# Medical-Image-Analysis-Laboratory/fetal_t2mapping

Measured on AMD Instinct MI355X. Metric: Mvoxel/s T2 fit, 256³×8TE 3-param LM, 1/2/4/8 GPU; % HBM roofline, higher is better.
Workload: dtype f64

## Files before the change

fetal_t2mapping_amd/csrc/t2fit_kernels.hip:

```cpp
#include <hip/hip_runtime.h>

#include <algorithm>
#include <atomic>
#include <cstdlib>
#include <string>

#include "t2fit_config.h"
#include "t2fit_diag.h"
#include "t2fit_dispatch.h"
#include "t2fit_error.h"
#include "t2fit_launch.h"
#include "t2fit_support.h"

using namespace t2fit;

namespace {

constexpr int kLdsStride = kBlock + 1;
#ifndef T2_SAMPLE_LOAD
#define T2_SAMPLE_LOAD(p) (*(p))
#endif
#ifndef T2_WAVE_HINT
#define T2_WAVE_HINT 2
#endif
// ... 209 lines not shown
        finite = finite && t2_finite(sv);
      }
    }
    ObjCtx c;
    c.P = &P;
    c.y = EchoView{col, kLoglinTile};
    double lb[3], ub[3];
    const bool feasible = lane_bounds(P, y0[q], lb, ub);
    LaneResult r;
    r.nit = 0; r.nfev = 0; r.fun = NAN;
    if (!feasible) {
      r.x[0] = NAN; r.x[1] = NAN; r.x[2] = 0.0;
      r.status = T2FIT_ST_INFEASIBLE;
    } else if (!finite) {
      r.x[0] = t2_clip(P.x0[0], lb[0], ub[0]); r.x[1] = t2_clip(P.x0[1], lb[1], ub[1]); r.x[2] = 0.0;
      r.status = T2FIT_ST_NONFINITE;
    } else {
      loglin_solve(c, lb, ub, want_fun, r);
    }
    LaneOutputs o;
    lane_epilogue(c, r, o, kExtras && m.r2 != nullptr, kExtras && m.se != nullptr);
    o_t2[q] = o.t2; o_k[q] = o.k; o_res[q] = o.res;
    if constexpr (kExtras) {
      if (m.r2) m.r2[v] = o.r2;
      if (m.se) m.se[v] = o.se;
      if (m.fun) m.fun[v] = o.fun;
      if (m.nit) m.nit[v] = o.nit;
      if (m.status) m.status[v] = o.status;
      if (m.xd) { m.xd[3 * v] = r.x[0]; m.xd[3 * v + 1] = r.x[1]; m.xd[3 * v + 2] = r.x[2]; }
      if (m.fund) m.fund[v] = r.fun;
    }
  }
  *reinterpret_cast<float4*>(m.t2 + v0) = make_float4(o_t2[0], o_t2[1], o_t2[2], o_t2[3]);
  *reinterpret_cast<float4*>(m.k + v0) = make_float4(o_k[0], o_k[1], o_k[2], o_k[3]);
  *reinterpret_cast<float4*>(m.sigma + v0) = make_float4(0.0f, 0.0f, 0.0f, 0.0f);
  *reinterpret_cast<float4*>(m.res + v0) = make_float4(o_res[0], o_res[1], o_res[2], o_res[3]);
}

constexpr int kChunkLarge = 256;
constexpr int kChunkSmall = 64;
constexpr int kQueueCap = 64 + kChunkLarge;

template <int MODEL, int NTE = 0, int HOME = PAIRS_LDS> struct LbfgsbLane {
  using Solver = Lbfgsb<MODEL, NTE, HOME>;
  using WaveWg = LbfgsbLane<MODEL, NTE, MODEL == T2FIT_MODEL_GAUSSIAN ? PAIRS_LDS
                                         : MODEL == T2FIT_MODEL_RICIAN ? PAIRS_GLOBAL : PAIRS_REG>;
  static constexpr bool kGlobalPart = Solver::kPairGlobal;
  static constexpr int NP = Solver::N;
  static constexpr int kNte = NTE;
  static constexpr int kHistDoubles = Solver::M * Solver::PAIR_L;
  static constexpr int kWavesPerSimd = 1;
  static constexpr bool kWaveWgOk = true;
#ifndef T2_WAVE_HINT_2PAR
#define T2_WAVE_HINT_2PAR 3
#endif
  static constexpr int kWaveWgHint = MODEL == T2FIT_MODEL_GAUSSIAN ? T2_WAVE_HINT_2PAR : kWaveHint;
  static constexpr int kRefillMin = MODEL == T2FIT_MODEL_RICIAN ? 4 : 8;
  static constexpr bool kSplit = true;
  __device__ static void init(Solver& s, const ObjCtx&, const double* x0, const double* lb, const double* ub,
                              double* hist, int hstride, double* ghist) { s.init(x0, lb, ub, hist, hstride, ghist, 64); }
  __device__ static void result(const Solver& s, const ObjCtx&, LaneResult& r) { s.result(r); }
  template <int J> __device__ static void take_sample(Solver& s, float y) {
    if constexpr (NTE > 0 && J < NTE) s.ys[J] = y;
  }
};
template <typename T, int NPAR, int NTE = 0> struct LmLaneAdaptor {
  using Solver = LmLane<T, NPAR, NTE>;
  using WaveWg = LmLaneAdaptor<T, NPAR, NTE>;
  static constexpr bool kGlobalPart = false;
  static constexpr int NP = NPAR;
  static constexpr int kNte = NTE;
  static constexpr int kHistDoubles = 0;
  static constexpr bool kWaveWgOk = false;
  static constexpr int kWaveWgHint = 1;
  static constexpr int kWavesPerSimd = sizeof(T) == 4 ? 4 : 1;
  static constexpr int kRefillMin = 24;
  static constexpr bool kSplit = false;
  __device__ static void init(Solver& s, const ObjCtx& c, const double* x0, const double* lb, const double* ub,
                              double*, int, double*) { s.init(c, x0, lb, ub); }
  __device__ static void result(const Solver& s, const ObjCtx& c, LaneResult& r) { s.result(c, r); }
  template <int J> __device__ static void take_sample(Solver&, float) {}
};

template <class A, int kChunk, bool kTrace, bool kExtras, int kWg = kBlock, bool kRegs = false>
__device__ __forceinline__ void persistent_fit(const LaneParams& P, const float* __restrict__ echoes, int layout,
                                               const uint8_t* __restrict__ mask, int64_t n_vox, const DevMaps& m,
                                               unsigned long long* next_chunk, int refill_min, int take, double* ghist_all) {
  extern __shared__ float lds[];
  constexpr int NP = A::NP;
  constexpr bool kWaveWg = kRegs;
  static_assert(kRegs ? (kChunk == 64 && A::kNte > 0 && A::kNte <= 8) : kWg == kBlock,
                "workgroup of 256 lanes, or waves taking 64-voxel chunks with the samples in registers");
  constexpr int kStride = kWaveWg ? 64 : kLdsStride;
  const int lane = threadIdx.x & 63, wave = threadIdx.x >> 6;
  float* col = lds + threadIdx.x;
  double* hist = reinterpret_cast<double*>(lds + (kWaveWg ? 0 : ((P.n_te * kStride + 1) & ~1))) + threadIdx.x;
  uint32_t* queue = reinterpret_cast<uint32_t*>(hist - threadIdx.x + A::kHistDoubles * kWg) + wave * kQueueCap;
  double* ghist = nullptr;
  if constexpr (A::kGlobalPart)
    ghist = ghist_all + ((size_t)blockIdx.x * (kWg / 64) + wave) * (A::Solver::M * 64) + lane;
  uint32_t qv = 0;
  const unsigned long long lt_mask = lane == 0 ? 0ull : (~0ull >> (64 - lane));
  const EchoView y{col, kStride};
  int q_head = 0, q_count = 0;
  bool chunks_left = true;
  bool busy = false, done = false;
  int64_t v = 0;
  typename A::Solver s;
  ObjCtx c;
  c.P = &P;
  c.y = y;
  double box_x0[3], box_lb[3], box_ub[3];
#pragma unroll
  for (int j = 0; j < 3; ++j) { box_x0[j] = P.x0[j]; box_lb[j] = P.lb[j]; box_ub[j] = P.ub[j]; }
  T2_STAMPS_BEGIN(queue - wave * kQueueCap + (kBlock / 64) * kQueueCap, wave, lane, c)
  T2_RECORD_PLACEMENT(next_chunk, blockIdx.x * (kWg / 64) + wave, lane)
  bool parked = false;
  int pend = 0;
  const int kTake = take;
  int64_t base_a = 0;
  int sub_a = 0;
  uint32_t idx_b = 0;
  uint8_t mask_a = 0;
  auto load_mask = [&](int64_t base) -> uint8_t {
    const int64_t vv = base + lane;
    return vv < n_vox ? (mask ? mask[vv] : (uint8_t)1) : (uint8_t)0;
  };
  if constexpr (kWaveWg) {
    uint32_t c0 = 0;
    if (lane == 0) c0 = (uint32_t)atomicAdd(next_chunk, 1ull);
    base_a = (int64_t)__shfl(c0, 0, 64) * (64 * kTake);
    mask_a = load_mask(base_a);
    if (lane == 0) idx_b = (uint32_t)atomicAdd(next_chunk, 1ull);
  }
  for (;;) {
    unsigned long long need = __ballot(!busy);
    if (__popcll(need) >= refill_min || need == ~0ull) {
      do {
      T2_BLK_T0(t_rf)
      if (done) {
        LaneResult r;
        A::result(s, c, r);
        store_fit<kExtras>(m, v, r);
        done = false;
      }
      bool fresh = false;
      if constexpr (kWaveWg) {
        unsigned long long want = need;
        for (;;) {
          if (q_count == 0) {
            if (!chunks_left) break;
            const int64_t base = base_a;
            if (base >= n_vox) { chunks_left = false; break; }
            const int64_t vv = base + lane;
            const bool act = mask_a != 0;
            if (++sub_a < kTake) {
              base_a += 64;
              mask_a = load_mask(base_a);
            } else {
              sub_a = 0;
              base_a = (int64_t)__shfl(idx_b, 0, 64) * (64 * kTake);
              mask_a = load_mask(base_a);
              if (lane == 0) idx_b = (uint32_t)atomicAdd(next_chunk, 1ull);
            }
            const unsigned long long b = __ballot(act);
            q_count = __popcll(b);
            q_head = 0;
            const int dst = act ? __popcll(b & lt_mask) : q_count + __popcll(~b & lt_mask);
            qv = (uint32_t)__builtin_amdgcn_ds_permute(dst << 2, (int)(uint32_t)vv);
            if (vv < n_vox && !act) store_masked<kExtras, true>(m, vv);
            if (q_count == 0) continue;
          }
          const int rank = __popcll(want & lt_mask);
          const uint32_t got = (uint32_t)__builtin_amdgcn_ds_bpermute(((q_head + rank) & 63) << 2, (int)qv);
          if (!busy && rank < q_count) {
            v = (int64_t)got;
            busy = true;
            fresh = true;
          }
          const int n_want = __popcll(want);
          const int taken = n_want < q_count ? n_want : q_count;
          q_head += taken;
          q_count -= taken;
          want = __ballot(!busy);
          if (want == 0ull) break;
        }
      } else {
      const int n_need = __popcll(need);
      while (q_count < n_need && chunks_left) {
        unsigned long long cidx = 0;
        if (lane == 0) cidx = atomicAdd(next_chunk, 1ull);
        cidx = __shfl(cidx, 0, 64);
        const int64_t base = (int64_t)cidx * kChunk;
        if (base >= n_vox) { chunks_left = false; break; }
        if (q_head != 0) {
          uint32_t tmp = 0;
          if (lane < q_count) tmp = queue[q_head + lane];
          if (lane < q_count) queue[lane] = tmp;
          q_head = 0;
        }
        bool act[kChunk / 64];
#pragma unroll
        for (int q = 0; q < kChunk / 64; ++q) {
          const int64_t vv = base + q * 64 + lane;
          act[q] = vv < n_vox && (mask == nullptr || mask[vv] != 0);
        }
#pragma unroll
        for (int q = 0; q < kChunk / 64; ++q) {
          const unsigned long long b = __ballot(act[q]);
          if (act[q]) queue[q_count + __popcll(b & lt_mask)] = (uint32_t)(base + q * 64 + lane);
          q_count += __popcll(b);
        }
#pragma unroll
        for (int q = 0; q < kChunk / 64; ++q) {
          const int64_t vv = base + q * 64 + lane;
          if (vv < n_vox && !act[q]) store_masked<kExtras, true>(m, vv);
        }
      }
      if (!busy) {
        const int rank = __popcll(need & lt_mask);
        if (rank < q_count) {
          v = (int64_t)queue[q_head + rank];
          busy = true;
          fresh = true;
        }
      }
      const int taken = n_need < q_count ? n_need : q_count;
      q_head += taken;
      q_count -= taken;
      }
      if (fresh) {
        bool finite = true;
        float ymax = 0.0f, y0 = 0.0f;
        const int n_te = A::kNte > 0 ? A::kNte : P.n_te;
        float first8[8] = {};
        for (int i0 = 0; i0 < n_te; i0 += 8) {
          float tmp[8];
#pragma unroll
          for (int j = 0; j < 8; ++j)
            if (i0 + j < n_te)
              tmp[j] = T2_SAMPLE_LOAD(layout == T2FIT_LAYOUT_TE_MAJOR ? &echoes[(int64_t)(i0 + j) * n_vox + v]
                                                                      : &echoes[v * n_te + (i0 + j)]);
#pragma unroll
          for (int j = 0; j < 8; ++j)
            if (i0 + j < n_te) {
              const float sv = tmp[j];
              if constexpr (!kWaveWg) col[(i0 + j) * kStride] = sv;
              if (i0 == 0) first8[j] = sv;
              finite = finite && t2_finite(sv);
              if (i0 + j == 0) { y0 = sv; ymax = sv; }
              ymax = sv > ymax ? sv : ymax;
            }
        }
        if (P.norm) {
          if constexpr (A::kNte > 0) {
#pragma unroll
            for (int j = 0; j < 8; ++j)
              if (j < n_te) {
                const float sv = first8[j] / ymax;
                first8[j] = sv;
                if constexpr (!kWaveWg) col[j * kStride] = sv;
                finite = finite && t2_finite(sv);
              }
          } else {
            for (int i = 0; i < n_te; ++i) {
              const float sv = col[i * kStride] / ymax;
              col[i * kStride] = sv;
              finite = finite && t2_finite(sv);
            }
          }
        }
        if constexpr (A::kNte > 0)
          static_for<0, 8>([&](auto JC) { A::template take_sample<decltype(JC)::value>(s, first8[decltype(JC)::value]); });
        double lb[3], ub[3];
#pragma unroll
        for (int j = 0; j < 3; ++j) { lb[j] = box_lb[j]; ub[j] = box_ub[j]; }
        if (P.no_prior) {
          lb[0] = (double)y0; ub[0] = P.np_k_ub;
          lb[1] = P.np_t2_lb; ub[1] = P.np_t2_ub;
        }
        bool feasible = true;
#pragma unroll
        for (int j = 0; j < NP; ++j) feasible = feasible && !(lb[j] > ub[j]);
        if (!feasible || !finite) {
          LaneResult r;
          r.nit = 0; r.nfev = 0; r.fun = NAN;
          for (int j = 0; j < 3; ++j)
            r.x[j] = !feasible ? (j < NP ? NAN : 0.0) : (j < NP ? t2_clip(box_x0[j], lb[j], ub[j]) : 0.0);
          r.status = !feasible ? T2FIT_ST_INFEASIBLE : T2FIT_ST_NONFINITE;
          store_fit<kExtras>(m, v, r);
          busy = false;
        } else {
          if constexpr (kTrace) {
            c.trace = m.trace + (size_t)v * 4 * m.trace_cap;
            c.trace_cap = m.trace_cap;
            c.trace_n = m.trace_len + v;
            *c.trace_n = 0;
          }
          A::init(s, c, box_x0, lb, ub, hist, kWg, ghist);
          if constexpr (A::kSplit) { T2_STAMPS_ATTACH(s) }
        }
      }
      T2_BLK_END(c, 8, t_rf)
      need = __ballot(!busy);
      } while (need == ~0ull && (chunks_left || q_count != 0));
    }
    if (__ballot(busy) == 0ull) break;
    if constexpr (A::kSplit) {
      if (busy) {
        if (!parked) {
          T2_BLK_T0(t_ev)
          s.eval(c);
          T2_BLK_END(c, 7, t_ev)
          pend = s.digest(c);
        }
        if (pend == A::Solver::GO_BEGIN || pend == A::Solver::GO_FAIL) {
          T2_BLK_T0(t_bg)
          pend = s.begin_pass(c, pend);
          T2_BLK_END(c, 9, t_bg)
        }
        parked = pend == A::Solver::GO_BEGIN || pend == A::Solver::GO_FAIL;
        if (pend == A::Solver::GO_DONE) { busy = false; done = true; }
      }
    } else {
      if (busy) s.eval(c);
      if (busy && s.advance(c)) {
        busy = false;
        done = true;
      }
    }
  }
  if (done) {
    LaneResult r;
    A::result(s, c, r);
    store_fit<kExtras>(m, v, r);
  }
  T2_STAMPS_END(next_chunk, lane)
}

template <class A, int kChunk, bool kTrace = false, int kWavesPerSimd = 1, bool kExtras = true, int kWg = kBlock,
          bool kRegs = false>
__global__ __launch_bounds__(kWg, kWavesPerSimd) void fit_persistent_kernel(const LaneParams P,
                                                                    const float* __restrict__ echoes, int layout,
                                                                    const uint8_t* __restrict__ mask, int64_t n_vox,
                                                                    DevMaps m, unsigned long long* next_chunk, int refill_min,
                                                                    int take, double* ghist) {
  persistent_fit<A, kChunk, kTrace, kExtras, kWg, kRegs>(P, echoes, layout, mask, n_vox, m, next_chunk, refill_min, take, ghist);
}

__global__ __launch_bounds__(kBlock) void residuals_kernel(const LaneParams P, const float* __restrict__ echoes,
                                                           int layout, const uint8_t* __restrict__ mask,
                                                           int64_t n_vox, const float* __restrict__ t2,
                                                           const float* __restrict__ k,
                                                           const float* __restrict__ sigma, float* res, float* r2,
                                                           float* se) {
  extern __shared__ float lds[];
  const int lane = threadIdx.x;
  const int64_t base = (int64_t)blockIdx.x * kBlock;
  const int64_t v = base + lane;
  const bool in_range = v < n_vox;
  const bool active = in_range && (mask == nullptr || mask[v] != 0);
  stage_echoes(lds, echoes, layout, P.n_te, n_vox, base, active);
  if (!in_range) return;
  float out = 0.0f, out2 = 0.0f, out3 = 0.0f;
  if (active) {
    bool finite;
    float y0_raw;
    const ObjCtx c = prepare_samples(P, lds + lane, kLdsStride, finite, y0_raw);
    const float kv = k[v], tv = t2[v], sv = sigma ? sigma[v] : 0.0f;
    out = residual_mean(c, kv, tv, sv);
    if (r2) out2 = r_squared(c, (double)kv, (double)tv, (double)sv);
    if (se) out3 = t2_std_error(c, (double)kv, (double)tv, (double)sv);
  }
  res[v] = out;
  if (r2) r2[v] = out2;
  if (se) se[v] = out3;
}

using FitKernel = void (*)(const LaneParams, const float*, int, const uint8_t*, int64_t, DevMaps);

FitKernel pick_kernel(const t2fit_config& c) {
  if (c.solver == T2FIT_SOLVER_LM) {
    if (c.precision == T2FIT_PREC_F32)
      return c.model == T2FIT_MODEL_GAUSSIAN
                 ? fit_volume_kernel<T2FIT_SOLVER_LM, T2FIT_PREC_F32, T2FIT_MODEL_GAUSSIAN>
                 : fit_volume_kernel<T2FIT_SOLVER_LM, T2FIT_PREC_F32, T2FIT_MODEL_GAUSSIAN_RICIAN>;
    return c.model == T2FIT_MODEL_GAUSSIAN
               ? fit_volume_kernel<T2FIT_SOLVER_LM, T2FIT_PREC_F64, T2FIT_MODEL_GAUSSIAN>
               : fit_volume_kernel<T2FIT_SOLVER_LM, T2FIT_PREC_F64, T2FIT_MODEL_GAUSSIAN_RICIAN>;
  }
  if (c.solver == T2FIT_SOLVER_LOGLIN)
    return fit_volume_kernel<T2FIT_SOLVER_LOGLIN, T2FIT_PREC_F64, T2FIT_MODEL_GAUSSIAN>;
  return nullptr;
}

bool wants_extras(const DevMaps& dm) { return dm.r2 || dm.se || dm.fun || dm.nit || dm.status || dm.xd || dm.fund; }

struct LaunchArgs {
  unsigned grid; size_t lds_samples; hipStream_t st;
  const LaneParams& P; const float* echoes; int layout; const uint8_t* mask; int64_t n_vox; const DevMaps& dm;
  unsigned long long* counter;
  bool big;
};

template <class A, bool kLargeOnly = false, bool kWaveOnly = false>
hipError_t launch_persistent(const LaunchArgs& a) {
  constexpr int W = A::kWavesPerSimd;
  const Tuning& tune = tuning();
  const DevMaps& dm = a.dm;
  const bool extras = wants_extras(dm);
  const int refill_min = tune.refill_min > 0 ? tune.refill_min : A::kRefillMin;
  if constexpr (!kPhaseStamps && kLargeOnly && A::kHistDoubles > 0 && A::kWaveWgOk) {
    if (tune.wave_wg) {
      using AW = typename A::WaveWg;
      constexpr int kHint = AW::kWaveWgHint;
      auto k64 = extras ? fit_persistent_kernel<AW, kChunkSmall, false, kHint, true, 64, true>
                        : fit_persistent_kernel<AW, kChunkSmall, false, kHint, false, 64, true>;
      unsigned wg = 64;
      if constexpr (kWgShapeDiag) {
        if (tune.wave_wg == 2) { k64 = fit_persistent_kernel<AW, kChunkSmall, false, 1, false, 256, true>; wg = 256; }
        if (tune.wave_wg == 3) { k64 = fit_persistent_kernel<AW, kChunkSmall, false, 1, false, 128, true>; wg = 128; }
      }
      size_t lds64 = (size_t)AW::kHistDoubles * wg * sizeof(double);
      unsigned per_cu = (unsigned)std::min<size_t>(wg == 64 ? 4 * kHint : 512 / wg, 128 / ceil_div<size_t>(lds64, 1280));
      if (tune.waves_per_cu > 0 && (unsigned)tune.waves_per_cu < per_cu) {
        per_cu = (unsigned)tune.waves_per_cu;
        lds64 = (size_t)(128 / per_cu) * 1280;
      }
      hipError_t e = hipFuncSetAttribute(reinterpret_cast<const void*>(k64), hipFuncAttributeMaxDynamicSharedMemorySize,
                                         (int)lds64);
// ... 211 lines not shown
```

fetal_t2mapping_amd/csrc/t2fit_lbfgsb.h:

```cpp
#pragma once

#include <type_traits>

#include "t2fit_lane.h"

namespace t2fit {

template <int MODEL> struct ObjTerm;
T2_HD double rician_log_term(float log_y, double log_s2, bool legacy) {
  return legacy ? (double)(log_y - (float)log_s2) : (double)log_y - log_s2;
}
template <> struct ObjTerm<T2FIT_MODEL_GAUSSIAN> {
  double k, t2;
  T2_HD void set(const ObjCtx&, const double* x) { k = x[0]; t2 = x[1]; }
  T2_HD double at(const ObjCtx& c, int i) const {
    const double r = (double)c.sample(i) - k * t2_exp_core(t2_fdiv(-c.P->te[i], t2));
    return r * r;
  }
  T2_HD double finish(const ObjCtx& c, double s) const { return s / c.P->n_te; }
};
template <> struct ObjTerm<T2FIT_MODEL_GAUSSIAN_RICIAN> {
  double k2, t2, s2;
  T2_HD void set(const ObjCtx&, const double* x) { k2 = x[0] * x[0]; t2 = x[1]; s2 = x[2] * x[2]; }
  T2_HD double at(const ObjCtx& c, int i) const {
// ... 36 lines not shown
    for (int j = 0; j < 8; ++j) r[j] = t.at(c, j);
    int i = 8;
    for (; i + 8 <= n; i += 8) {
      T2_UNROLL
      for (int j = 0; j < 8; ++j) r[j] += t.at(c, i + j);
    }
    s = ((r[0] + r[1]) + (r[2] + r[3])) + ((r[4] + r[5]) + (r[6] + r[7]));
    for (; i < n; ++i) s += t.at(c, i);
  }
  return t.finish(c, s);
}

enum { LS_START = 0, LS_FG = 1, LS_CONV = 2, LS_WARN = 3, LS_ERROR = 4 };

struct LsState {
  int task, stage;
  bool brackt;
  double ginit, gtest, gx, gy, finit, fx, fy, stx, sty, stmin, stmax, width, width1;
};

T2_HD double lb_max(double a, double b) { return __builtin_fmax(a, b); }
T2_HD double lb_min(double a, double b) { return __builtin_fmin(a, b); }
T2_HD double lb_abs(double a) { return __builtin_fabs(a); }
T2_HD double t2_max3(double a, double b, double c) { return lb_max(a, lb_max(b, c)); }

T2_HD void dcstep(double& stx, double& fx, double& dx, double& sty, double& fy, double& dy, double& stp,
                  double fp, double dp, bool& brackt, double stpmin, double stpmax) {
  const double sgnd = !(dx < 0.0 || dx > 0.0) ? (double)NAN : (dx < 0.0 ? -dp : dp);
  const bool c1 = fp > fx;
  const bool c2 = !c1 && sgnd < 0.0;
  const bool c3 = !c1 && !c2 && lb_abs(dp) < lb_abs(dx);
  const bool c4 = !c1 && !c2 && !c3;
  const double sta = c4 ? sty : stx, fa = c4 ? fy : fx, da = c4 ? dy : dx;
  const double theta = t2_fdiv(3.0 * (fa - fp), stp - sta) + da + dp;
  const double s = t2_max3(lb_abs(theta), lb_abs(da), lb_abs(dp));
  const double rs = t2_rcp_for_div(s);
  const double ts = t2_div_by_rcp(theta, s, rs);
  double arg = ts * ts - t2_div_by_rcp(da, s, rs) * t2_div_by_rcp(dp, s, rs);
  arg = c3 ? lb_max(0.0, arg) : arg;
  double gamma = s * t2_sqrt_core(arg);
  const bool lt_x = stp < stx, gt_x = stp > stx, gt_y = stp > sty;
  const bool flip = (c1 & lt_x) | (!c1 & ((c4 & gt_y) | (!c4 & gt_x)));
  gamma = flip ? -gamma : gamma;
  const double gd1 = c1 ? dx : dp;
  const double p = (gamma - gd1) + theta;
  const double q3 = (gamma + (dx - dp)) + gamma, gd2 = c1 ? dp : (c2 ? dx : dy), q124 = ((gamma - gd1) + gamma) + gd2;
  const double q = c3 ? q3 : q124;
  const double r = t2_fdiv(p, q);
  const double far_end = gt_x ? stpmax : stpmin;
  const double stpc1 = stx + r * (stp - stx), stpc234 = stp + r * (sta - stp);
  double stpc = c1 ? stpc1 : stpc234;
  const bool r_neg = r < 0.0, g_nz = gamma != 0.0;
  stpc = (c3 & !(r_neg & g_nz)) ? far_end : stpc;
  const double qden1 = t2_fdiv(fx - fp, stp - stx) + dx, qden23 = dp - dx;
  const double qden = c1 ? qden1 : qden23;
  const double qq = t2_fdiv(c1 ? dx : dp, qden);
  const double quad = c1 ? qq * 0.5 : qq;
  const double stpq1 = stx + quad * (stp - stx), stpq23 = stp + quad * (stx - stp);
  const double stpq = c1 ? stpq1 : stpq23;
  const double dc = lb_abs(stpc - stp), dq = lb_abs(stpq - stp);
  const double f1 = lb_abs(stpc - stx) < lb_abs(stpq - stx) ? stpc : stpc + (stpq - stpc) * 0.5;
  const double farther = dc > dq ? stpc : stpq, nearer = dc < dq ? stpc : stpq;
  const double lim = stp + 0.66 * (sty - stp);
  const double f3lo = lb_min(lim, nearer), f3hi = lb_max(lim, nearer);
  const double f3b = gt_x ? f3lo : f3hi;
  const double f3u = lb_max(stpmin, lb_min(stpmax, farther));
  const double f4 = brackt ? stpc : far_end;
  const double stpf = c1 ? f1 : (c2 ? farther : (c3 ? (brackt ? f3b : f3u) : f4));
  brackt = brackt || c1 || c2;
  const bool swap = !c1 && sgnd < 0.0;
  const double nsty = c1 ? stp : (swap ? stx : sty);
  const double nfy = c1 ? fp : (swap ? fx : fy);
  const double ndy = c1 ? dp : (swap ? dx : dy);
  const double nstx = c1 ? stx : stp;
  const double nfx = c1 ? fx : fp;
  const double ndx = c1 ? dx : dp;
  sty = nsty; fy = nfy; dy = ndy;
  stx = nstx; fx = nfx; dx = ndx;
  stp = stpf;
}

T2_HD void dcsrch_start(double f, double g, double stp, double ftol, double stpmin, double stpmax, LsState& s) {
  const double xtrapu = 4.0;
  const bool bad = stp < stpmin || stp > stpmax || g >= 0.0;
  s.brackt = false;
  s.stage = 1;
  s.finit = f; s.ginit = g; s.gtest = ftol * s.ginit;
  s.width = stpmax - stpmin; s.width1 = s.width * 2.0;
  s.stx = 0.0; s.fx = s.finit; s.gx = s.ginit;
  s.sty = 0.0; s.fy = s.finit; s.gy = s.ginit;
  s.stmin = 0.0; s.stmax = stp + xtrapu * stp;
  s.task = bad ? LS_ERROR : LS_FG;
}

T2_HD int dcsrch_tests(double f, double g, double stp, double gtol, double xtol, double stpmin, double stpmax,
                       LsState& s) {
  const double ftest = s.finit + stp * s.gtest;
  const bool f_ok = f <= ftest, g_pos = g >= 0.0, g_le = g <= s.gtest, g_ge = g >= s.gtest;
  s.stage = ((s.stage == 1) & f_ok & g_pos) ? 2 : s.stage;
  const bool outside = (stp <= s.stmin) | (stp >= s.stmax);
  const bool narrow = s.stmax - s.stmin <= xtol * s.stmax;
  const bool at_max = (stp == stpmax) & f_ok & g_le;
  const bool at_min = (stp == stpmin) & ((f > ftest) | g_ge);
  const bool conv = f_ok & (lb_abs(g) <= gtol * (-s.ginit));
  const int task = conv ? LS_CONV : (((s.brackt & (outside | narrow)) | at_max | at_min) ? LS_WARN : LS_FG);
  s.task = task;
  return task;
}

T2_HD void dcsrch_update(double f, double g, double& stp, double xtol, double stpmin, double stpmax, LsState& s) {
  const double xtrapl = 1.1, xtrapu = 4.0, p5 = 0.5, p66 = 0.66;
  const double ftest = s.finit + stp * s.gtest;
  const bool modified = (s.stage == 1) & (f <= s.fx) & (f > ftest);
  const double gt = modified ? s.gtest : 0.0;
  double fm = modified ? f - stp * gt : f, gm = modified ? g - gt : g;
  double fxm = modified ? s.fx - s.stx * gt : s.fx, fym = modified ? s.fy - s.sty * gt : s.fy;
  double gxm = modified ? s.gx - gt : s.gx, gym = modified ? s.gy - gt : s.gy;
  dcstep(s.stx, fxm, gxm, s.sty, fym, gym, stp, fm, gm, s.brackt, s.stmin, s.stmax);
  s.fx = modified ? fxm + s.stx * gt : fxm;
  s.fy = modified ? fym + s.sty * gt : fym;
  s.gx = modified ? gxm + gt : gxm;
  s.gy = modified ? gym + gt : gym;
  const double span = lb_abs(s.sty - s.stx);
  const double mid = s.stx + p5 * (s.sty - s.stx);
  stp = (s.brackt & (span >= p66 * s.width1)) ? mid : stp;
  s.width1 = s.brackt ? s.width : s.width1;
  s.width = s.brackt ? span : s.width;
  const double lo_b = lb_min(s.stx, s.sty), hi_b = lb_max(s.stx, s.sty);
  const double lo_u = stp + xtrapl * (stp - s.stx), hi_u = stp + xtrapu * (stp - s.stx);
  s.stmin = s.brackt ? lo_b : lo_u;
  s.stmax = s.brackt ? hi_b : hi_u;
  stp = lb_max(stp, stpmin);
  stp = lb_min(stp, stpmax);
  const bool stuck = s.brackt & ((stp <= s.stmin) | (stp >= s.stmax) | (s.stmax - s.stmin <= xtol * s.stmax));
  stp = stuck ? s.stx : stp;
  s.task = LS_FG;
}

T2_HD void dcsrch(double f, double g, double& stp, double gtol, double xtol, double stpmin, double stpmax,
                  LsState& s) {
  if (dcsrch_tests(f, g, stp, gtol, xtol, stpmin, stpmax, s) == LS_FG) dcsrch_update(f, g, stp, xtol, stpmin, stpmax, s);
}

struct NpSum {
  double seq = 0.0, p0 = 0.0, p1 = 0.0, p2 = 0.0, s = 0.0;
  template <int J> T2_HD void add(double t) {
    seq = J == 0 ? 0.0 + t : seq + t;
    if constexpr (J == 0) p0 = t;
    else if constexpr (J == 1) p0 += t;
    else if constexpr (J == 2) p1 = t;
    else if constexpr (J == 3) { p1 += t; p0 += p1; }
    else if constexpr (J == 4) p1 = t;
    else if constexpr (J == 5) p1 += t;
    else if constexpr (J == 6) p2 = t;
    else { p2 += t; p1 += p2; s = p0 + p1; }
  }
  T2_HD void tail(double t) { s += t; }
  T2_HD double total(int n) const { return n < 8 ? seq : s; }
};


template <int NTE> struct RowSums4 {
  static constexpr bool kGeneral = NTE == 0, kTree = NTE == 8;
  double s[kTree ? 1 : 4];
  double p[kTree ? 4 : 1], q[kTree ? 4 : 1], h[kTree ? 4 : 1];
  double r[kGeneral ? 8 : 1][4];
  T2_HD void init() {
// ... 70 lines not shown
  double* hist;
  double* ghist;
  int hstride, gstride, head;
  int iwhere[N];
  int col, nit, nfev, ifun;
  uint8_t status;
  bool first;
  bool wn_stale;
  float ys[NTE > 0 ? NTE : 1];
  T2_HD float smp(const ObjCtx& c, int i) const {
    if constexpr (NTE > 0) return ys[i];
    else return c.sample(i);
  }
  T2_DIAG_COUNTERS
#if !defined(__HIPCC__)
  int n_reset = 0;
#define T2_COUNT_RESET() ++n_reset
#else
#define T2_COUNT_RESET()
#endif

  T2_HD void eval(const ObjCtx& c) {
    const LaneParams& P = *c.P;
    const int n = NTE > 0 ? NTE : P.n_te;
    double x1[N], dx[N];
    T2_UNROLL
    for (int i = 0; i < N; ++i) {
      double h = P.fd_step;
      if ((x[i] + h) - x[i] == 0.0)
        h = 1.4901161193847656e-08 * (x[i] >= 0 ? 1.0 : -1.0) * lb_max(1.0, lb_abs(x[i]));
      const double lower = x[i] - lb[i], upper = ub[i] - x[i];
      const double xs = x[i] + h;
      const bool violated = (xs < lb[i]) | (xs > ub[i]);
      const bool fitting = lb_abs(h) <= lb_max(lower, upper);
      h = (violated & fitting) ? -h : h;
      const double h_far = upper >= lower ? upper : -lower;
      h = fitting ? h : h_far;
      x1[i] = x[i] + h;
      dx[i] = x1[i] - x[i];
    }
    nfev += 1 + N;
    if (MODEL != T2FIT_MODEL_RICIAN && n >= 16) {
      f = objective_t<MODEL>(c, x);
      T2_UNROLL
      for (int i = 0; i < N; ++i) {
        double xt[N];
        T2_UNROLL
        for (int j = 0; j < N; ++j) xt[j] = j == i ? x1[j] : x[j];
        g[i] = (objective_t<MODEL>(c, xt) - f) / dx[i];
      }
      return;
    }
    NpSum s0, s1, s2, s3;
    const double nd = (double)n, inv_n = P.inv_n;
    auto mean = [&](double sum) { return t2_div_by_rcp(sum, nd, inv_n); };
    if constexpr (MODEL == T2FIT_MODEL_GAUSSIAN) {
      const double k = x[0], t2 = x[1], kp = x1[0], t2p = x1[1];
      const double rt2 = t2_rcp_for_div(t2), rt2p = t2_rcp_for_div(t2p);
      auto body = [&](int i, auto add) {
        const double y = (double)smp(c, i), te = P.te[i];
        const double E = t2_exp_core(t2_div_by_rcp(-te, t2, rt2)), Ep = t2_exp_core(t2_div_by_rcp(-te, t2p, rt2p));
        const double r0 = y - k * E, r1 = y - kp * E, r2 = y - k * Ep;
        add(r0 * r0, r1 * r1, r2 * r2, 0.0);
      };
      static_for<0, 8>([&](auto JC) {
        constexpr int J = decltype(JC)::value;
        if (J < n) body(J, [&](double a, double b2, double c2, double) { s0.add<J>(a); s1.add<J>(b2); s2.add<J>(c2); });
      });
      for (int i = 8; i < n; ++i) body(i, [&](double a, double b2, double c2, double) { s0.tail(a); s1.tail(b2); s2.tail(c2); });
      f = mean(s0.total(n));
      g[0] = t2_fdiv(mean(s1.total(n)) - f, dx[0]);
      g[1] = t2_fdiv(mean(s2.total(n)) - f, dx[1]);
    } else if constexpr (MODEL == T2FIT_MODEL_GAUSSIAN_RICIAN) {
      const double k2 = x[0] * x[0], kp2 = x1[0] * x1[0], t2 = x[1], t2p = x1[1];
      const double sg2 = x[N - 1] * x[N - 1], sgp2 = x1[N - 1] * x1[N - 1];
      const double rt2 = t2_rcp_for_div(t2), rt2p = t2_rcp_for_div(t2p);
      const double tol = 0x1p-22;
      const bool near_k = 2.0 * lb_abs(dx[0]) <= tol * lb_abs(x[0]), near_s = 2.0 * lb_abs(dx[N - 1]) <= tol * lb_abs(x[N - 1]);
      const bool near_t = 2.0 * P.te_max * lb_abs(dx[1]) <= tol * (t2 * t2p), s_pos = sg2 > 0.0;
      const bool near = near_k & near_s & near_t & s_pos;
      if (T2_WAVE_ANY(!near)) {
        RowSums4<NTE> sums;
        sums.init();
        T2_NOUNROLL
        for (int i = 0; i < n; ++i) {
          float yf;
          if constexpr (NTE > 0) {
            yf = ys[0];
            T2_UNROLL
            for (int j = 0; j + 1 < NTE; ++j) ys[j] = ys[j + 1];
            ys[NTE - 1] = yf;
          } else {
            yf = c.sample(i);
          }
          const double y = (double)yf, te = P.te[i];
          const double E = t2_exp_core(t2_div_by_rcp(-2.0 * te, t2, rt2)), Ep = t2_exp_core(t2_div_by_rcp(-2.0 * te, t2p, rt2p));
          const double r0 = y - t2_sqrt_core(k2 * E + sg2), r1 = y - t2_sqrt_core(kp2 * E + sg2);
          const double r2 = y - t2_sqrt_core(k2 * Ep + sg2), r3 = y - t2_sqrt_core(k2 * E + sgp2);
          const double tm[4] = {r0 * r0, r1 * r1, r2 * r2, r3 * r3};
          sums.add(i, n, tm);
        }
        f = mean(sums.total(0));
        g[0] = t2_fdiv(mean(sums.total(1)) - f, dx[0]);
        g[1] = t2_fdiv(mean(sums.total(2)) - f, dx[1]);
        g[N - 1] = t2_fdiv(mean(sums.total(3)) - f, dx[N - 1]);
        return;
      }
      auto body = [&](int i, auto add) {
        const double y = (double)smp(c, i), te = P.te[i];
        const double E = t2_exp_core(t2_div_by_rcp(-2.0 * te, t2, rt2)), Ep = t2_exp_core(t2_div_by_rcp(-2.0 * te, t2p, rt2p));
        double h;
        const double q0 = t2_sqrt_core_h(k2 * E + sg2, h);
        const double r0 = y - q0, r1 = y - t2_sqrt_near(kp2 * E + sg2, h);
        const double r2 = y - t2_sqrt_near(k2 * Ep + sg2, h), r3 = y - t2_sqrt_near(k2 * E + sgp2, h);
        add(r0 * r0, r1 * r1, r2 * r2, r3 * r3);
      };
      static_for<0, 8>([&](auto JC) {
        constexpr int J = decltype(JC)::value;
        if (J < n) body(J, [&](double a, double b2, double c2, double d2) { s0.add<J>(a); s1.add<J>(b2); s2.add<J>(c2); s3.add<J>(d2); });
      });
      for (int i = 8; i < n; ++i) body(i, [&](double a, double b2, double c2, double d2) { s0.tail(a); s1.tail(b2); s2.tail(c2); s3.tail(d2); });
      f = mean(s0.total(n));
      g[0] = t2_fdiv(mean(s1.total(n)) - f, dx[0]);
      g[1] = t2_fdiv(mean(s2.total(n)) - f, dx[1]);
      g[N - 1] = t2_fdiv(mean(s3.total(n)) - f, dx[N - 1]);
    } else {
      const double k = x[0], kp = x1[0], t2 = x[1], t2p = x1[1];
      const double sg2 = x[N - 1] * x[N - 1], sgp2 = x1[N - 1] * x1[N - 1];
      const double ls2 = t2_log(sg2), lsp2 = t2_log(sgp2);
      const double rt2 = t2_rcp_for_div(t2), rt2p = t2_rcp_for_div(t2p);
      const double rs2 = t2_rcp_for_div(sg2), rsp2 = t2_rcp_for_div(sgp2);
      const bool legacy = P.numpy_legacy != 0;
      const double tol = 0x1p-22;
      const bool near_lane = 2.0 * lb_abs(dx[0]) <= tol * lb_abs(x[0]) && 2.0 * lb_abs(dx[N - 1]) <= tol * lb_abs(x[N - 1]) &&
                             2.0 * P.te_max * lb_abs(dx[1]) <= tol * (t2 * t2p);
      const bool near = !T2_WAVE_ANY(!near_lane);
      RowSums4<NTE> sums;
      sums.init();
      T2_NOUNROLL
      for (int i = 0; i < n; ++i) {
        float yf;
        if constexpr (NTE > 0) {
          yf = ys[0];
          T2_UNROLL
          for (int j = 0; j + 1 < NTE; ++j) ys[j] = ys[j + 1];
          ys[NTE - 1] = yf;
        } else {
          yf = c.sample(i);
        }
        const double te = P.te[i];
        const double E = t2_exp_core(t2_div_by_rcp(-te, t2, rt2)), Ep = t2_exp_core(t2_div_by_rcp(-te, t2p, rt2p));
        const double yd = (double)yf, y2 = (double)(yf * yf);
        const float ly = logf(yf);
        const double m[4] = {k * E, kp * E, k * Ep, k * E};
        double xx[4], li[4], tm[4];
        T2_UNROLL
        for (int j = 0; j < 4; ++j) xx[j] = t2_div_by_rcp(m[j] * yd, j == 3 ? sgp2 : sg2, j == 3 ? rsp2 : rs2);
        t2_log_i0e4(xx, li, near);
        T2_UNROLL
        for (int j = 0; j < 4; ++j) {
          const double a = rician_log_term(ly, j == 3 ? lsp2 : ls2, legacy);
          const double b = t2_div_by_rcp(y2 + m[j] * m[j], 2.0 * (j == 3 ? sgp2 : sg2), 0.5 * (j == 3 ? rsp2 : rs2));
          const double dd = (xx[j] < 0 ? -xx[j] : xx[j]) + li[j];
          tm[j] = (a - b) + dd;
        }
        sums.add(i, n, tm);
      }
      f = -sums.total(0);
      g[0] = t2_fdiv(-sums.total(1) - f, kp - k);
      g[1] = t2_fdiv(-sums.total(2) - f, t2p - t2);
      g[N - 1] = t2_fdiv(-sums.total(3) - f, dx[N - 1]);
    }
  }

  T2_HD double projgr(const double* x, const double* g) const {
    double nrm = 0.0;
    T2_UNROLL
    for (int i = 0; i < N; ++i) {
      double gi = g[i];
      const double g_up = lb_max(x[i] - ub[i], gi), g_lo = lb_min(x[i] - lb[i], gi);
      gi = gi < 0.0 ? g_up : g_lo;
      nrm = lb_max(nrm, lb_abs(gi));
    }
    return nrm;
  }

  T2_HD int slot_of(int p) const { return (head + p) % M; }
  T2_HD double& hratio(int q, int e) const {
    if constexpr (kPairGlobal) {
      if (e == N - 2) return ghist[q * gstride];
    }
    return hist[(q * PAIR_L + e) * hstride];
  }
  T2_HD double& hy(int q, int i) const { return hist[(q * PAIR_L + (kSplit ? N - 2 : N - 1) + i) * hstride]; }
  T2_HD void load_s(int q, double* sv) const {
    sv[0] = 1.0;
    T2_UNROLL
    for (int i = 1; i < (kPairRegs ? N - 1 : N); ++i) sv[i] = hratio(q, i - 1);
    if constexpr (kPairRegs) {
      const int at = M - col + (q - head + M) % M;
      double v = this->hr[0];
      static_for<1, M>([&](auto IC) { v = at == decltype(IC)::value ? this->hr[decltype(IC)::value] : v; });
      sv[N - 1] = v;
    }
  }
  T2_HD void store_s(int q, const double* sv) {
    double big = lb_abs(sv[0]);
    T2_UNROLL
    for (int i = 1; i < N; ++i) big = lb_max(big, lb_abs(sv[i]));
    const double least = big * 0x1p-400;
    const double p0 = lb_abs(sv[0]) < least ? (sv[0] < 0.0 ? -least : least) : sv[0];
    const double r = t2_rcp_for_div(p0);
    T2_UNROLL
    for (int i = 1; i < (kPairRegs ? N - 1 : N); ++i) hratio(q, i - 1) = t2_div_by_rcp(sv[i], p0, r);
    if constexpr (kPairRegs) {
      T2_UNROLL
      for (int i = 0; i + 1 < M; ++i) this->hr[i] = this->hr[i + 1];
      this->hr[M - 1] = t2_div_by_rcp(sv[N - 1], p0, r);
    }
  }

  T2_HD void build_b(double (*B)[N]) const {
    double U[N][N];
    T2_UNROLL
    for (int i = 0; i < N; ++i)
      T2_UNROLL
      for (int j = 0; j < N; ++j) U[i][j] = i == j ? theta : 0.0;
    double rp[2][N], yp[2][N];
    T2_UNROLL
    for (int i = 0; i < N; ++i) { rp[0][i] = 0.0; yp[0][i] = 0.0; rp[1][i] = 0.0; yp[1][i] = 0.0; }
    if constexpr (kPairRegs) {
      auto fetch = [&](int qs, int set) {
        T2_UNROLL
        for (int i = 1; i < N - 1; ++i) rp[set][i] = hratio(qs, i - 1);
        T2_UNROLL
        for (int i = 0; i < N; ++i) yp[set][i] = hy(qs, i);
      };
      int q = head + col;
      q = q >= M ? q - M : q;
      fetch(q, 0);
      static_for<0, M>([&](auto IC) {
        constexpr int t = decltype(IC)::value, cur = t & 1, nxt = cur ^ 1;
        if constexpr (t + 1 < M) {
          q = q + 1 == M ? 0 : q + 1;
          fetch(q, nxt);
        }
        if (t >= M - col) {
          rp[cur][N - 1] = this->hr[t];
          double bs[N];
          T2_UNROLL
          for (int i = 0; i < N; ++i) {
            double a = U[0][i];
            T2_UNROLL
            for (int j = 1; j < N; ++j) a = fma(j >= i ? U[i][j] : U[j][i], rp[cur][j], a);
            bs[i] = a;
          }
          double sbs = bs[0];
          T2_UNROLL
          for (int i = 1; i < N; ++i) sbs = fma(rp[cur][i], bs[i], sbs);
          const double rsbs = t2_fast_rcp(sbs);
          double tb[N];
          T2_UNROLL
          for (int i = 0; i < N; ++i) tb[i] = bs[i] * rsbs;
          T2_UNROLL
          for (int i = 0; i < N; ++i)
            T2_UNROLL
            for (int j = i; j < N; ++j) U[i][j] = fma(yp[cur][i], yp[cur][j], fma(-bs[i], tb[j], U[i][j]));
        }
      });
    } else {
      int q = head;
      if (col > 0) {
        T2_UNROLL
        for (int i = 1; i < N; ++i) rp[0][i] = hratio(q, i - 1);
        T2_UNROLL
        for (int i = 0; i < N; ++i) yp[0][i] = hy(q, i);
      }
      static_for<0, M>([&](auto PC) {
        constexpr int p = decltype(PC)::value, cur = p & 1, nxt = cur ^ 1;
        if (p < col) {
          const int step = q + 1 == M ? 0 : q + 1;
          const int qn = (!kPairGlobal || p + 1 < col) ? step : q;
          q = qn;
          T2_UNROLL
          for (int i = 1; i < N; ++i) rp[nxt][i] = hratio(qn, i - 1);
          T2_UNROLL
          for (int i = 0; i < N; ++i) yp[nxt][i] = hy(qn, i);
          double bs[N];
          T2_UNROLL
          for (int i = 0; i < N; ++i) {
            double a = U[0][i];
            T2_UNROLL
            for (int j = 1; j < N; ++j) a = fma(j >= i ? U[i][j] : U[j][i], rp[cur][j], a);
            bs[i] = a;
          }
          double sbs = bs[0];
          T2_UNROLL
          for (int i = 1; i < N; ++i) sbs = fma(rp[cur][i], bs[i], sbs);
          const double rsbs = t2_fast_rcp(sbs);
          double tb[N];
          T2_UNROLL
          for (int i = 0; i < N; ++i) tb[i] = bs[i] * rsbs;
          T2_UNROLL
          for (int i = 0; i < N; ++i)
            T2_UNROLL
            for (int j = i; j < N; ++j) U[i][j] = fma(yp[cur][i], yp[cur][j], fma(-bs[i], tb[j], U[i][j]));
        }
      });
    }
    T2_UNROLL
    for (int i = 0; i < N; ++i)
      T2_UNROLL
      for (int j = 0; j < N; ++j) B[i][j] = j >= i ? U[i][j] : U[j][i];
  }

  T2_HD void cauchy(const double* x, const double* g, const double (*B)[N], double theta, double sbgnrm,
                    int* iwhere, double* xcp) const {
    const double epsmch = 2.220446049250313e-16;
    T2_UNROLL
    for (int i = 0; i < N; ++i) xcp[i] = x[i];
    const bool live = sbgnrm > 0.0;
    double d[N], tbk[N], zfix[N];
    bool hasbk[N];
    int nbreak = 0;
    double f1 = 0.0;
    T2_UNROLL
    for (int i = 0; i < N; ++i) {
      const double neggi = -g[i];
      const double tl = x[i] - lb[i], tu = ub[i] - x[i];
// ... 237 lines not shown
      nit = nit1;
      if (c.trace && *c.trace_n < c.trace_cap) {
        double* tr = c.trace + 4 * (*c.trace_n)++;
        tr[0] = x[0]; tr[1] = x[1]; tr[2] = N == 3 ? x[N - 1] : 0.0; tr[3] = f;
      }
    }
    if (iterate_on) {
      T2_UNROLL
      for (int i = 0; i < N; ++i) { r[i] = rn[i]; d[i] = dn[i]; }
    }
    if (store_pair) {
      if (col == M) {
        head = (head + 1) % M;
        col = M - 1;
      }
      const int q = slot_of(col);
      store_s(q, dn);
      T2_UNROLL
      for (int i = 0; i < N; ++i) hy(q, i) = rn[i] * rsy;
      ++col;
      theta = theta_n;
    }
    if ((was_first || newit) && converged && !(newit && out_of_budget)) status = T2FIT_ST_CONVERGED;
    const int next_ls = ifun - 1 >= P.maxls ? GO_FAIL : GO_TRIAL;
    const int next_it = (converged | (!was_first & out_of_budget)) ? GO_DONE : GO_BEGIN;
    const int next = cont ? next_ls : next_it;
    T2_BLK_END(c, 0, t_dig)
    set_trial(next == GO_TRIAL);
    return next;
  }

  T2_HD void set_trial(bool on = true) {
    T2_UNROLL
    for (int i = 0; i < N; ++i) {
      const double xt = stp * d[i] + t[i];
      x[i] = on ? (stp == 1.0 ? z[i] : xt) : x[i];
    }
  }

  T2_HD int begin_pass(const ObjCtx& c, int next) {
    const LaneParams& P = *c.P;
    bool ended = false;
    if (next == GO_FAIL) {
      T2_UNROLL
      for (int i = 0; i < N; ++i) { x[i] = t[i]; g[i] = r[i]; }
      f = fold;
      ended = col == 0;
      col = 0; theta = 1.0; wn_stale = false;
      T2_COUNT_RESET();
    }
    double B[N][N];
    T2_BLK_T0(t_b)
    build_b(B);
    T2_BLK_END(c, 3, t_b)
    T2_BLK_T0(t_c)
    cauchy(x, g, B, theta, sbgnrm, iwhere, z);
    T2_BLK_END(c, 4, t_c)
    int nfree = 0;
    T2_UNROLL
    for (int i = 0; i < N; ++i) nfree += iwhere[i] <= 0;
    bool restart = false;
    if (nfree != 0 && col != 0) {
      restart = wn_stale;
      if (!restart) {
        T2_BLK_T0(t_s)
        restart = !subsm(x, g, B, iwhere, z);
        T2_BLK_END(c, 5, t_s)
      }
    } else if (col != 0) {
      wn_stale = true;
    }
    if (restart) {
      wn_stale = false;
      col = 0; theta = 1.0;
      T2_COUNT_RESET();
    }
    T2_BLK_T0(t_l)
    T2_UNROLL
    for (int i = 0; i < N; ++i) { d[i] = z[i] - x[i]; t[i] = x[i]; r[i] = g[i]; }
    stpmx = 1e10;
    T2_UNROLL
    for (int i = 0; i < N; ++i) {
      const double a1 = d[i];
      const double a2 = (a1 < 0.0 ? lb[i] : ub[i]) - x[i];
      const bool at_bound = a1 < 0.0 ? a2 >= 0.0 : a2 <= 0.0;
      const bool limits = a1 < 0.0 ? a1 * stpmx < a2 : a1 * stpmx > a2;
      const double q = t2_fdiv(a2, a1);
      const double cand = at_bound ? 0.0 : (limits ? q : stpmx);
      stpmx = a1 != 0.0 ? cand : stpmx;
    }
    stpmx = nit == 0 ? 1.0 : stpmx;
    stp = 1.0;
    fold = f;
    gd = 0.0;
    T2_UNROLL
    for (int i = 0; i < N; ++i) gd += g[i] * d[i];
    gdold = gd;
    dcsrch_start(f, gd, stp, 1e-3, 0.0, stpmx, ls);
    ifun = 1;
    T2_BLK_END(c, 6, t_l)
    const int out = ended ? GO_DONE : (restart ? GO_BEGIN : ((ls.task != LS_FG || ifun - 1 >= P.maxls) ? GO_FAIL : GO_TRIAL));
    set_trial(out == GO_TRIAL);
    return out;
  }

  T2_HD bool advance(const ObjCtx& c) {
    int next = digest(c);
    while (next == GO_BEGIN || next == GO_FAIL) next = begin_pass(c, next);
    return next == GO_DONE;
  }

  T2_HD void result(LaneResult& out) const {
    T2_UNROLL
    for (int i = 0; i < 3; ++i) out.x[i] = 0.0;
    T2_UNROLL
    for (int i = 0; i < N; ++i) out.x[i] = x[i];
    out.fun = f;
    out.nit = nit;
    out.nfev = nfev;
    out.status = status;
  }
};

template <int MODEL>
T2_HD void lbfgsb_solve(const ObjCtx& c, const double* lb, const double* ub, LaneResult& out) {
  Lbfgsb<MODEL> s;
  double hist[Lbfgsb<MODEL>::M * Lbfgsb<MODEL>::PAIR] = {};
  s.init(c.P->x0, lb, ub, hist, 1);
  do {
    s.eval(c);
  } while (!s.advance(c));
  s.result(out);
}

}
```

Baseline: 1625.

## Reload fit parameters from kernarg segment and flatten solver branch logic

The persistent kernel no longer keeps the box bounds and initial guess in registers for its whole lifetime. It re-reads them through a scalar kernarg pointer, hidden behind an opaque asm barrier, each time a lane takes a new voxel, which is meant to lower register pressure. Several other local changes come along with it. The L-BFGS-B history fetch now uses precomputed offsets instead of a modular queue index, the echo samples are copied to a local array before the rotation loop, and the line-search bound tests are rewritten as branch-free boolean expressions. These add scalar loads per voxel refill and slightly change the stpmx edge-case semantics.

```diff
diff --git a/fetal_t2mapping_amd/csrc/t2fit_kernels.hip b/fetal_t2mapping_amd/csrc/t2fit_kernels.hip
--- a/fetal_t2mapping_amd/csrc/t2fit_kernels.hip
+++ b/fetal_t2mapping_amd/csrc/t2fit_kernels.hip
@@ -315,10 +315,12 @@
   template <int J> __device__ static void take_sample(Solver&, float) {}
 };
 
+using KernargParams = const __attribute__((address_space(4))) LaneParams*;
+
 template <class A, int kChunk, bool kTrace, bool kExtras, int kWg = kBlock, bool kRegs = false>
 __device__ __forceinline__ void persistent_fit(const LaneParams& P, const float* __restrict__ echoes, int layout,
                                                const uint8_t* __restrict__ mask, int64_t n_vox, const DevMaps& m,
-                                               unsigned long long* next_chunk, int refill_min, int take, double* ghist_all) {
+                                               unsigned long long* next_chunk, int refill_min, int take, double* ghist_all, KernargParams Pk) {
   extern __shared__ float lds[];
   constexpr int NP = A::NP;
   constexpr bool kWaveWg = kRegs;
@@ -343,9 +345,11 @@
   ObjCtx c;
   c.P = &P;
   c.y = y;
-  double box_x0[3], box_lb[3], box_ub[3];
-#pragma unroll
-  for (int j = 0; j < 3; ++j) { box_x0[j] = P.x0[j]; box_lb[j] = P.lb[j]; box_ub[j] = P.ub[j]; }
+  auto refill_params = [Pk] {
+    auto kp = Pk;
+    asm volatile("" : "+s"(kp));
+    return kp;
+  };
   T2_STAMPS_BEGIN(queue - wave * kQueueCap + (kBlock / 64) * kQueueCap, wave, lane, c)
   T2_RECORD_PLACEMENT(next_chunk, blockIdx.x * (kWg / 64) + wave, lane)
   bool parked = false;
@@ -485,7 +489,8 @@
               ymax = sv > ymax ? sv : ymax;
             }
         }
-        if (P.norm) {
+        const auto* const Pr = refill_params();
+        if (Pr->norm) {
           if constexpr (A::kNte > 0) {
 #pragma unroll
             for (int j = 0; j < 8; ++j)
@@ -505,12 +510,12 @@
         }
         if constexpr (A::kNte > 0)
           static_for<0, 8>([&](auto JC) { A::template take_sample<decltype(JC)::value>(s, first8[decltype(JC)::value]); });
-        double lb[3], ub[3];
-#pragma unroll
-        for (int j = 0; j < 3; ++j) { lb[j] = box_lb[j]; ub[j] = box_ub[j]; }
-        if (P.no_prior) {
-          lb[0] = (double)y0; ub[0] = P.np_k_ub;
-          lb[1] = P.np_t2_lb; ub[1] = P.np_t2_ub;
+        double box_x0[3], lb[3], ub[3];
+#pragma unroll
+        for (int j = 0; j < 3; ++j) { box_x0[j] = Pr->x0[j]; lb[j] = Pr->lb[j]; ub[j] = Pr->ub[j]; }
+        if (Pr->no_prior) {
+          lb[0] = (double)y0; ub[0] = Pr->np_k_ub;
+          lb[1] = Pr->np_t2_lb; ub[1] = Pr->np_t2_ub;
         }
         bool feasible = true;
 #pragma unroll
@@ -518,6 +523,7 @@
         if (!feasible || !finite) {
           LaneResult r;
           r.nit = 0; r.nfev = 0; r.fun = NAN;
+#pragma unroll
           for (int j = 0; j < 3; ++j)
             r.x[j] = !feasible ? (j < NP ? NAN : 0.0) : (j < NP ? t2_clip(box_x0[j], lb[j], ub[j]) : 0.0);
           r.status = !feasible ? T2FIT_ST_INFEASIBLE : T2FIT_ST_NONFINITE;
@@ -578,7 +584,8 @@
                                                                     const uint8_t* __restrict__ mask, int64_t n_vox,
                                                                     DevMaps m, unsigned long long* next_chunk, int refill_min,
                                                                     int take, double* ghist) {
-  persistent_fit<A, kChunk, kTrace, kExtras, kWg, kRegs>(P, echoes, layout, mask, n_vox, m, next_chunk, refill_min, take, ghist);
+  persistent_fit<A, kChunk, kTrace, kExtras, kWg, kRegs>(P, echoes, layout, mask, n_vox, m, next_chunk, refill_min, take, ghist,
+                                                         (KernargParams)__builtin_amdgcn_kernarg_segment_ptr());
 }
 
 __global__ __launch_bounds__(kBlock) void residuals_kernel(const LaneParams P, const float* __restrict__ echoes,
diff --git a/fetal_t2mapping_amd/csrc/t2fit_lbfgsb.h b/fetal_t2mapping_amd/csrc/t2fit_lbfgsb.h
--- a/fetal_t2mapping_amd/csrc/t2fit_lbfgsb.h
+++ b/fetal_t2mapping_amd/csrc/t2fit_lbfgsb.h
@@ -142,7 +142,8 @@
 
 T2_HD void dcsrch_start(double f, double g, double stp, double ftol, double stpmin, double stpmax, LsState& s) {
   const double xtrapu = 4.0;
-  const bool bad = stp < stpmin || stp > stpmax || g >= 0.0;
+  const bool below = stp < stpmin, above = stp > stpmax, uphill = g >= 0.0;
+  const bool bad = below | above | uphill;
   s.brackt = false;
   s.stage = 1;
   s.finit = f; s.ginit = g; s.gtest = ftol * s.ginit;
@@ -379,14 +380,19 @@
       if (T2_WAVE_ANY(!near)) {
         RowSums4<NTE> sums;
         sums.init();
+        float yr[NTE > 0 ? NTE : 1];
+        if constexpr (NTE > 0) {
+          T2_UNROLL
+          for (int j = 0; j < NTE; ++j) yr[j] = ys[j];
+        }
         T2_NOUNROLL
         for (int i = 0; i < n; ++i) {
           float yf;
           if constexpr (NTE > 0) {
-            yf = ys[0];
+            yf = yr[0];
             T2_UNROLL
-            for (int j = 0; j + 1 < NTE; ++j) ys[j] = ys[j + 1];
-            ys[NTE - 1] = yf;
+            for (int j = 0; j + 1 < NTE; ++j) yr[j] = yr[j + 1];
+            yr[NTE - 1] = yf;
           } else {
             yf = c.sample(i);
           }
@@ -527,21 +533,21 @@
     T2_UNROLL
     for (int i = 0; i < N; ++i) { rp[0][i] = 0.0; yp[0][i] = 0.0; rp[1][i] = 0.0; yp[1][i] = 0.0; }
     if constexpr (kPairRegs) {
-      auto fetch = [&](int qs, int set) {
-        T2_UNROLL
-        for (int i = 1; i < N - 1; ++i) rp[set][i] = hratio(qs, i - 1);
-        T2_UNROLL
-        for (int i = 0; i < N; ++i) yp[set][i] = hy(qs, i);
+      const int slot = PAIR_L * hstride;
+      const int q0r = head + col, q0 = q0r >= M ? q0r - M : q0r;
+      const int ia = q0 * slot, ib = ia - M * slot;
+      auto fetch = [&](auto TC, int set) {
+        constexpr int tf = decltype(TC)::value;
+        const double* p = (tf == 0 || q0 < M - tf) ? hist + (ia + tf * slot) : hist + (ib + tf * slot);
+        T2_UNROLL
+        for (int i = 1; i < N - 1; ++i) rp[set][i] = p[(i - 1) * hstride];
+        T2_UNROLL
+        for (int i = 0; i < N; ++i) yp[set][i] = p[(N - 2 + i) * hstride];
       };
-      int q = head + col;
-      q = q >= M ? q - M : q;
-      fetch(q, 0);
+      fetch(std::integral_constant<int, 0>{}, 0);
       static_for<0, M>([&](auto IC) {
         constexpr int t = decltype(IC)::value, cur = t & 1, nxt = cur ^ 1;
-        if constexpr (t + 1 < M) {
-          q = q + 1 == M ? 0 : q + 1;
-          fetch(q, nxt);
-        }
+        if constexpr (t + 1 < M) fetch(std::integral_constant<int, t + 1>{}, nxt);
         if (t >= M - col) {
           rp[cur][N - 1] = this->hr[t];
           double bs[N];
@@ -945,12 +951,14 @@
     T2_UNROLL
     for (int i = 0; i < N; ++i) {
       const double a1 = d[i];
-      const double a2 = (a1 < 0.0 ? lb[i] : ub[i]) - x[i];
-      const bool at_bound = a1 < 0.0 ? a2 >= 0.0 : a2 <= 0.0;
-      const bool limits = a1 < 0.0 ? a1 * stpmx < a2 : a1 * stpmx > a2;
+      const bool dec = a1 < 0.0, moves = a1 != 0.0;
+      const double a2 = (dec ? lb[i] : ub[i]) - x[i];
+      const double a2m = dec ? -a2 : a2;
+      const bool at_bound = moves & (a2m <= 0.0);
+      const bool limits = moves & (lb_abs(a1) * stpmx > a2m);
       const double q = t2_fdiv(a2, a1);
-      const double cand = at_bound ? 0.0 : (limits ? q : stpmx);
-      stpmx = a1 != 0.0 ? cand : stpmx;
+      const double lim = limits ? q : stpmx;
+      stpmx = at_bound ? 0.0 : lim;
     }
     stpmx = nit == 0 ? 1.0 : stpmx;
     stp = 1.0;
@@ -962,7 +970,9 @@
     dcsrch_start(f, gd, stp, 1e-3, 0.0, stpmx, ls);
     ifun = 1;
     T2_BLK_END(c, 6, t_l)
-    const int out = ended ? GO_DONE : (restart ? GO_BEGIN : ((ls.task != LS_FG || ifun - 1 >= P.maxls) ? GO_FAIL : GO_TRIAL));
+    const bool ls_off = ls.task != LS_FG, ls_spent = ifun - 1 >= P.maxls;
+    const int out_ls = (ls_off | ls_spent) ? GO_FAIL : GO_TRIAL;
+    const int out = ended ? GO_DONE : (restart ? GO_BEGIN : out_ls);
     set_trial(out == GO_TRIAL);
     return out;
   }
```

After: 1663, median of 6. 2.3% higher.
